# googleinterns/multimodal-long-transformer-2021

Measured on AMD Instinct MI355X. Metric: train-step samples/sec + attention TFLOPS, 4096-tok seq, higher is better.
Workload: dtype bf16; 1 GPU; BASELINE config 3: BERT-base dims, S=4096 (2+63^2 patches+125 text), radius 64 + 8 global tokens, bf16, per-GPU batch 4; step=train_step, per_gpu_batch=4, global_batch=4, seq_len=4096, parallelism=dp1, ranks_seen=1, params=111009852, optimizer=AdamW (fused flat step, bf16 shadow weights) + polynomial lr, clip 1.0, grad_allreduce=none (1 GPU), grad_reduce=mean, step_launch=HIP graph replay (recorded after 3 eager steps)

## Files before the change

include/mmt_layer.h:

```cpp
#ifndef MMT_LAYER_H_
#define MMT_LAYER_H_

#include <stddef.h>
#include <stdint.h>

#ifdef __cplusplus
extern "C" {
#endif

typedef struct mmt_rows_desc {
  int64_t rows;
  int32_t H;
  int32_t dtype;
  float eps;
  float dropout_p;
  uint64_t dropout_seed;
  int32_t accumulate;
  int32_t defer_reduce;
  const uint64_t* dropout_epoch;
} mmt_rows_desc;

size_t mmt_layer_workspace_bytes(const mmt_rows_desc* desc);

int mmt_ln_fwd(const mmt_rows_desc* desc, const void* x, const float* gamma, const float* beta,
// ... 107 lines not shown
                  void* workspace, size_t workspace_bytes, void* stream);

int mmt_embed_fwd_packed(const mmt_embed_desc* desc, const int32_t* word_ids, const int32_t* seg_ids,
                         const float* word_table, const float* seg_table, const float* pos_table ,
                         int32_t pos_rows, const float* gamma, const float* beta, const void* patch_proj ,
                         const float* patch_bias , const int32_t* example_starts,
                         const int32_t* patch_slots, int32_t n_examples, void* out, float* mean, float* rstd,
                         void* stream);
int mmt_embed_bwd_packed(const mmt_embed_desc* desc, const void* dout, const int32_t* sorted_ids,
                         const int32_t* order, const float* word_table, const float* gamma, const float* mean,
                         const float* rstd, float* dword_table, float* dgamma, float* dbeta, void* dpatch,
                         const int32_t* example_starts, const int32_t* patch_slots, int32_t n_examples,
                         void* workspace, size_t workspace_bytes, void* stream);

int mmt_xent_fwd(int64_t rows, int32_t C, int32_t dtype, const void* logits, int64_t ld,
                 const int32_t* labels, float* loss, float* lse, void* stream);
int mmt_xent_fwd_argmax(int64_t rows, int32_t C, int32_t dtype, const void* logits, int64_t ld,
                        const int32_t* labels, float* loss, float* lse, int32_t* argmax, void* stream);
int mmt_xent_bwd(int64_t rows, int32_t C, int32_t dtype, const void* logits, int64_t ld,
                 const int32_t* labels, const float* lse, const float* coef, void* dlogits, int64_t ldd,
                 void* stream);
int mmt_xent_bwd_scaled(int64_t rows, int32_t C, int32_t dtype, const void* logits, int64_t ld,
                        const int32_t* labels, const float* lse, const float* coef, const float* gscale,
                        void* dlogits, int64_t ldd, void* stream);
int mmt_weighted_loss(int64_t rows, const float* loss, const float* weight, const float* lmul, const float* mask,
                      int64_t mask_div, float* out3, float* coef, void* stream);

void mmt_ffn_set_cu_budget(int32_t cus);
int mmt_ffn_gelu_gemm(const void* x, int64_t ldx, const void* w, int64_t ldw, const float* bias, void* u,
                      int64_t ldu, void* g, int64_t ldg, int64_t M, int64_t N, int64_t K, void* stream);
int mmt_ffn_dgelu_gemm(const void* dy, int64_t lddy, const void* w, int64_t ldw, const void* u, int64_t ldu,
                       const float* bias, void* du, int64_t lddu, int64_t M, int64_t N, int64_t K, void* stream);

typedef struct mmt_image_desc {
  int32_t B;
  int32_t image_size;
  int32_t patch_size;
  int32_t out_dtype;
  int32_t channel_bits;
  float mean[3];
} mmt_image_desc;

int mmt_image_patches(const mmt_image_desc* desc, const uint8_t* pixels, int64_t pixels_bytes, const int64_t* offsets,
                      const int32_t* heights, const int32_t* widths, const uint8_t* flip, void* normalised_out,
                      float* unnormalised_out, int32_t* label_ids_out, void* stream);

#ifdef __cplusplus
}
#endif
#endif
```

multimodal-long-transformer-2021_amd/csrc/ffn_gemm.hip:

```cpp
#include "../../include/mmt_attn.h"
#include "../../include/mmt_layer.h"
#include "attn_tile.h"
#include "layer_common.h"
#include "mmt_err.h"

#include <atomic>

namespace mmt {

struct FfnGemmParams {
  const __bf16* a;
  const __bf16* b;
  const float* bias;
  const __bf16* u_in;
  __bf16* u_out;
  __bf16* d;
  long lda, ldb, ldu, ldd;
  int M, N, K, tiles_m, tiles_n, tiles_per_wg;
};

static std::atomic<int> g_ffn_cus{256};
static int cu_budget() { return g_ffn_cus.load(std::memory_order_relaxed); }

constexpr int kFfnStage = 64 * 1024;
enum { kEpiBias = 0, kEpiGelu = 1, kEpiDgelu = 2 };

__device__ __forceinline__ void ffn_wait_dma() { asm volatile("s_waitcnt vmcnt(0)" ::: "memory"); }

template <int BT, int EPI>
__global__ __launch_bounds__(512, 2) void ffn_gemm_kernel(const FfnGemmParams p) {
  extern __shared__ __attribute__((aligned(16))) unsigned char smem[];
  const int tid = threadIdx.x, lane = tid & 63;
  const int wave = __builtin_amdgcn_readfirstlane(tid >> 6);
  const int h = lane >> 5, li = lane & 15, cb = (lane >> 4) & 1, r = lane & 31;
  int t_begin, t_end;
  {
    const int nwg = gridDim.x, b = blockIdx.x, x = b & 7;
    const int base = nwg >> 3, rem = nwg & 7;
    const int L = x * base + min(x, rem) + (b >> 3);
    t_begin = L * p.tiles_per_wg;
    t_end = min(p.tiles_m * p.tiles_n, t_begin + p.tiles_per_wg);
  }
  if (t_begin >= t_end) return;
  const int n_steps = p.K >> 6;

  const bool is_a = wave < 4;
  const int drow = lane >> 3, dpos = lane & 7;
  const __bf16* gsrc[8];
#pragma unroll
  for (int j = 0; j < 8; ++j) {
    const int idx = wave * 8 + j;
    const int rg = idx & 3, row = rg * 8 + drow;
    if (idx < 32 || BT == 1) {
      const int t8 = (idx >> 2) & 7;
      const int ch = dpos ^ ((row >> 1) & 7);
      gsrc[j] = (idx < 32 ? p.a + (long)(t8 * 32 + row) * p.lda : p.b + (long)(t8 * 32 + row) * p.ldb) + ch * 8;
    } else {
      const int i2 = idx - 32, kslab = i2 >> 4, t4 = (i2 >> 2) & 3;
      const int ch = (((dpos >> 2) ^ ((row >> 1) & 1)) << 2) | (dpos & 3);
      gsrc[j] = p.b + (long)(kslab * 32 + row) * p.ldb + t4 * 64 + ch * 8;
    }
  }
  const long sstep = is_a ? 64 : (BT == 1 ? 64 : 64 * p.ldb);
  const long tstep_m = is_a ? 256 * p.lda : 0, tstep_n = is_a ? 0 : (BT == 1 ? 256 * p.ldb : 256);
  const unsigned lds0 = (unsigned)(size_t)(__attribute__((address_space(3))) unsigned char*)smem;
  auto dma = [&](unsigned stage, int tm, int tn, int step) {
    const long off = tm * tstep_m + tn * tstep_n + step * sstep;
#pragma unroll
    for (int j = 0; j < 8; ++j) glds16(gsrc[j] + off, stage + (wave * 8 + j) * 1024);
  };

  const int wm = wave & 3, wn = wave >> 2;
  const int arow = r * 128, ax = (r >> 1) & 7;
  const int frow = 8 * h + (li >> 2);
  int fo[2];
#pragma unroll
  for (int db = 0; db < 2; ++db) fo[db] = frow * 128 + ((db ^ ((frow >> 1) & 1)) << 6) + 32 * cb + 8 * (li & 3);
  const int erow = lane >> 3, ech = lane & 7;

  int tm = t_begin / p.tiles_n, tn = t_begin - tm * p.tiles_n;
  dma(lds0, tm, tn, 0);
  ffn_wait_dma();
  __syncthreads();
  int gs = 0;

  for (int t = t_begin; t < t_end; ++t) {
    int tm_next = tm, tn_next = tn + 1;
    if (tn_next == p.tiles_n) { tn_next = 0; ++tm_next; }
    f32x16 acc[2][4];
#pragma unroll
    for (int a = 0; a < 2; ++a)
#pragma unroll
      for (int b = 0; b < 4; ++b) acc[a][b] = f32x16{0};

    const int m0 = tm * 256, n0 = tn * 256;
    bf16x8 uq[3][4];
    auto load_u = [&](int blk, bf16x8 (&dst)[4]) {
      const __bf16* up = p.u_in + (long)(m0 + wm * 64 + (blk & 1) * 32 + erow) * p.ldu + n0 + wn * 128 + (blk >> 1) * 64 + ech * 8;
#pragma unroll
// ... 14 lines not shown
        for (int a = 0; a < 2; ++a)
          af[a] = *reinterpret_cast<const bf16x8*>(cur + (wm * 2 + a) * 4096 + arow + coff);
#pragma unroll
        for (int b = 0; b < 4; ++b) {
          if (BT == 1) {
            bfr[b] = *reinterpret_cast<const bf16x8*>(cur + 32768 + (wn * 4 + b) * 4096 + arow + coff);
          } else {
            const unsigned char* base = cur + 32768 + ((s >> 1) * 4 + wn * 2 + (b >> 1)) * 4096 + fo[b & 1] + (s & 1) * 2048;
            const bf16x4 lo = __builtin_bit_cast(bf16x4, __builtin_amdgcn_ds_read_tr16_b64_v4i16((__attribute__((address_space(3))) s16x4*)(base)));
            const bf16x4 hi = __builtin_bit_cast(bf16x4, __builtin_amdgcn_ds_read_tr16_b64_v4i16((__attribute__((address_space(3))) s16x4*)(base + 512)));
#pragma unroll
            for (int j = 0; j < 4; ++j) { bfr[b][j] = lo[j]; bfr[b][4 + j] = hi[j]; }
          }
        }
#pragma unroll
        for (int a = 0; a < 2; ++a)
#pragma unroll
          for (int b = 0; b < 4; ++b)
            acc[a][b] = __builtin_amdgcn_mfma_f32_32x32x16_bf16(af[a], bfr[b], acc[a][b], 0, 0, 0);
      }
      ffn_wait_dma();
      __syncthreads();
    }

    float* park = reinterpret_cast<float*>(smem + ((gs - 1) & 1) * kFfnStage + wave * 8192);
#pragma unroll
    for (int blk = 0; blk < 4; ++blk) {
      const int hb = blk >> 1, a = blk & 1;
      const int ncol = n0 + wn * 128 + hb * 64 + ech * 8;
      const int mrow0 = m0 + wm * 64 + a * 32;
      float bs[8];
#pragma unroll
      for (int j = 0; j < 8; ++j) bs[j] = 0.f;
      if (p.bias) load_param(p.bias + ncol, bs);
      if (EPI == kEpiDgelu && blk + 2 < 4) load_u(blk + 2, uq[(blk + 2) % 3]);
#pragma unroll
      for (int b2 = 0; b2 < 2; ++b2)
#pragma unroll
        for (int i = 0; i < 16; ++i) park[kap(i, h) * 64 + 32 * b2 + r] = acc[a][2 * hb + b2][i];
      __builtin_amdgcn_fence(__ATOMIC_ACQ_REL, "wavefront");
      __builtin_amdgcn_wave_barrier();
#pragma unroll
      for (int it = 0; it < 4; ++it) {
        const int row = it * 8 + erow;
        float v[8];
        Chunk<float>::load(park + row * 64 + ech * 8, v);
        const long orow = (long)(mrow0 + row);
        if (EPI == kEpiDgelu) {
          const bf16x8 uu = uq[blk % 3][it];
#pragma unroll
          for (int j = 0; j < 8; j += 2) {
            f32x2 dz;
            (void)gelu_tanh_x2(f32x2{(float)uu[j] + bs[j], (float)uu[j + 1] + bs[j + 1]}, dz);
            v[j] *= dz[0]; v[j + 1] *= dz[1];
          }
        } else {
#pragma unroll
          for (int j = 0; j < 8; ++j) v[j] += bs[j];
          if (EPI == kEpiGelu) {
            if (p.u_out) Chunk<__bf16>::store(p.u_out + orow * p.ldu + ncol, v);
#pragma unroll
            for (int j = 0; j < 8; j += 2) {
              f32x2 dz;
              const f32x2 gz = gelu_tanh_x2(f32x2{v[j], v[j + 1]}, dz);
              v[j] = gz[0]; v[j + 1] = gz[1];
            }
          }
        }
        Chunk<__bf16>::store(p.d + orow * p.ldd + ncol, v);
      }
      __builtin_amdgcn_fence(__ATOMIC_ACQ_REL, "wavefront");
      __builtin_amdgcn_wave_barrier();
    }
    if (t + 1 < t_end) __syncthreads();
    tm = tm_next; tn = tn_next;
  }
}

template <int BT, int EPI>
static hipError_t launch_ffn(const FfnGemmParams& p_in, hipStream_t st) {
  FfnGemmParams p = p_in;
  const int tiles = p.tiles_m * p.tiles_n, cus = cu_budget();
  p.tiles_per_wg = (tiles + cus - 1) / cus;
  const int grid = (tiles + p.tiles_per_wg - 1) / p.tiles_per_wg;
  const int lds = 2 * kFfnStage;
  (void)hipFuncSetAttribute(reinterpret_cast<const void*>(ffn_gemm_kernel<BT, EPI>), hipFuncAttributeMaxDynamicSharedMemorySize, lds);
  hipLaunchKernelGGL((ffn_gemm_kernel<BT, EPI>), dim3(grid), dim3(512), lds, st, p);
  return hipGetLastError();
}


static int ffn_check(const char* who, const void* a, const void* b, const void* d, int64_t M, int64_t N, int64_t K,
                     int64_t lda, int64_t ldb, int64_t ldb_min, int64_t ldd) {
  if (!a || !b || !d) return fail(MMT_E_INVALID, "%s: NULL argument", who);
  if (M <= 0 || N <= 0 || K <= 0 || (M % 256) || (N % 256) || (K % 64) || M > (1 << 30) || N > (1 << 30) || K > (1 << 30))
    return fail(MMT_E_UNSUPPORTED, "%s: needs M %% 256 == 0, N %% 256 == 0, K %% 64 == 0 (got %lld, %lld, %lld)", who,
                (long long)M, (long long)N, (long long)K);
  if ((lda % 8) || (ldb % 8) || (ldd % 8) || lda < K || ldb < ldb_min || ldd < N) return fail(MMT_E_INVALID, "%s: bad leading dimensions", who);
  if (((uintptr_t)a & 15) || ((uintptr_t)b & 15) || ((uintptr_t)d & 15)) return fail(MMT_E_INVALID, "%s: operands must be 16-byte aligned", who);
  return MMT_OK;
}

}

extern "C" void mmt_ffn_set_cu_budget(int32_t cus) {
  mmt::g_ffn_cus.store(cus < 32 ? 32 : (cus > 256 ? 256 : cus), std::memory_order_relaxed);
}

extern "C" int mmt_ffn_gelu_gemm(const void* x, int64_t ldx, const void* w, int64_t ldw, const float* bias, void* u,
                                 int64_t ldu, void* g, int64_t ldg, int64_t M, int64_t N, int64_t K, void* stream) {
  int rc = mmt::ffn_check("mmt_ffn_gelu_gemm", x, w, g, M, N, K, ldx, ldw, K, ldg);
  if (rc != MMT_OK) return rc;
  if (u && ((ldu % 8) || ldu < N || ((uintptr_t)u & 15))) return mmt::fail(MMT_E_INVALID, "mmt_ffn_gelu_gemm: bad u");
  if (bias && ((uintptr_t)bias & 15)) return mmt::fail(MMT_E_INVALID, "mmt_ffn_gelu_gemm: bias must be 16-byte aligned");
  mmt::FfnGemmParams p{};
  p.a = (const __bf16*)x; p.b = (const __bf16*)w; p.bias = bias; p.u_out = (__bf16*)u; p.d = (__bf16*)g;
  p.lda = ldx; p.ldb = ldw; p.ldu = ldu; p.ldd = ldg; p.M = (int)M; p.N = (int)N; p.K = (int)K;
  p.tiles_m = (int)(M / 256); p.tiles_n = (int)(N / 256);
  const hipError_t e = mmt::launch_ffn<1, mmt::kEpiGelu>(p, (hipStream_t)stream);
  return e == hipSuccess ? MMT_OK : mmt::fail(MMT_E_LAUNCH, "mmt_ffn_gelu_gemm: %s", hipGetErrorString(e));
}

extern "C" int mmt_ffn_dgelu_gemm(const void* dy, int64_t lddy, const void* w, int64_t ldw, const void* u, int64_t ldu,
                                  const float* bias, void* du, int64_t lddu, int64_t M, int64_t N, int64_t K, void* stream) {
  int rc = mmt::ffn_check("mmt_ffn_dgelu_gemm", dy, w, du, M, N, K, lddy, ldw, N, lddu);
  if (rc != MMT_OK) return rc;
  if (!u || (ldu % 8) || ldu < N || ((uintptr_t)u & 15)) return mmt::fail(MMT_E_INVALID, "mmt_ffn_dgelu_gemm: bad u");
  if (bias && ((uintptr_t)bias & 15)) return mmt::fail(MMT_E_INVALID, "mmt_ffn_dgelu_gemm: bias must be 16-byte aligned");
  mmt::FfnGemmParams p{};
  p.a = (const __bf16*)dy; p.b = (const __bf16*)w; p.bias = bias; p.u_in = (const __bf16*)u; p.d = (__bf16*)du;
  p.lda = lddy; p.ldb = ldw; p.ldu = ldu; p.ldd = lddu; p.M = (int)M; p.N = (int)N; p.K = (int)K;
  p.tiles_m = (int)(M / 256); p.tiles_n = (int)(N / 256);
  const hipError_t e = mmt::launch_ffn<0, mmt::kEpiDgelu>(p, (hipStream_t)stream);
  return e == hipSuccess ? MMT_OK : mmt::fail(MMT_E_LAUNCH, "mmt_ffn_dgelu_gemm: %s", hipGetErrorString(e));
}
```

multimodal-long-transformer-2021_amd/mmt_amd/_lib.py:

```python
from __future__ import annotations

import ctypes
import os
import subprocess

_HERE = os.path.dirname(os.path.abspath(__file__))
_CSRC = os.path.join(os.path.dirname(_HERE), 'csrc')
LIB_PATH = os.path.join(_HERE, 'libmmt_attn.so')

MMT_ABI_VERSION = 4
MMT_F32, MMT_BF16 = 0, 1
MMT_IDS_NONE, MMT_IDS_1D, MMT_IDS_2D = 0, 1, 2
MMT_IDS_2D_IMAGE = 3
MMT_FLAG_SCALE_BEFORE_ADD = 1
MMT_FLAG_ACCUM_REL_GRADS = 2
MMT_FLAG_EXAMPLE_IDS = 4
MMT_FLAG_EXAMPLE_STARTS = 8


def image_grid(radius: int, start: int) -> int:
  return (int(radius) & 0xFF) | ((int(start) & 0x7FFFFF) << 8)

MMT_TUNE_FWD_WALK = 0x01
MMT_TUNE_FWD_PWIN = 0x100
MMT_TUNE_FWD_ROWS_ONE_WG = 0x200
MMT_TUNE_FWD_NO_WIN = 0x02
MMT_TUNE_FWD_FORCE_WIN = 0x04
MMT_TUNE_BWD_NO_HANDOVER = 0x08
MMT_TUNE_BWD_HO_PER_WAVE = 0x10
MMT_TUNE_BWD_NO_PEEL_DQ = 0x20
MMT_TUNE_BWD_NO_PEEL_DKV = 0x40
MMT_TUNE_BWD_DQ_PLANE_MAJOR = 0x80

EXPORTS = ('mmt_abi_version', 'mmt_last_error', 'mmt_write_step_scalars', 'mmt_workspace_bytes', 'mmt_attn_fwd',
           'mmt_attn_bwd', 'mmt_side_inputs',
           'mmt_layer_workspace_bytes', 'mmt_ln_fwd', 'mmt_ln_bwd', 'mmt_residual_block_fwd',
           'mmt_residual_block_bwd', 'mmt_bias_gelu_fwd', 'mmt_bias_gelu_bwd', 'mmt_colsum_reduce', 'mmt_colsum_reduce_batch', 'mmt_accumulate_grad', 'mmt_grad_clip_scale', 'mmt_adamw_step', 'mmt_wgrad_accumulate',
           'mmt_wgrad_bias_accumulate', 'mmt_wgrad_grouped', 'mmt_wgrad_group_workspace_bytes', 'mmt_wgrad_workspace_bytes', 'mmt_wgrad_set_cu_budget', 'mmt_embed_fwd', 'mmt_embed_bwd', 'mmt_embed_fwd_packed', 'mmt_embed_bwd_packed',
           'mmt_embed_workspace_bytes', 'mmt_xent_fwd', 'mmt_xent_fwd_argmax', 'mmt_xent_bwd', 'mmt_xent_bwd_scaled', 'mmt_weighted_loss', 'mmt_colsum', 'mmt_colsum_workspace_bytes', 'mmt_ln_bwd_add', 'mmt_ffn_gelu_gemm', 'mmt_ffn_dgelu_gemm', 'mmt_ffn_set_cu_budget',
           'mmt_image_patches')


class EmbedDesc(ctypes.Structure):
  _fields_ = [('rows', ctypes.c_int64), ('S', ctypes.c_int32), ('H', ctypes.c_int32), ('dtype', ctypes.c_int32),
              ('vocab', ctypes.c_int32), ('seg_vocab', ctypes.c_int32), ('patch_start', ctypes.c_int32),
              ('n_patch', ctypes.c_int32), ('eps', ctypes.c_float), ('dropout_p', ctypes.c_float),
              ('accumulate', ctypes.c_int32), ('dropout_seed', ctypes.c_uint64), ('dropout_epoch', ctypes.c_void_p)]


class RowsDesc(ctypes.Structure):
  _fields_ = [('rows', ctypes.c_int64), ('H', ctypes.c_int32), ('dtype', ctypes.c_int32),
              ('eps', ctypes.c_float), ('dropout_p', ctypes.c_float),
              ('dropout_seed', ctypes.c_uint64), ('accumulate', ctypes.c_int32),
              ('defer_reduce', ctypes.c_int32), ('dropout_epoch', ctypes.c_void_p)]


class MaskDesc(ctypes.Structure):
  _fields_ = [('valid_len', ctypes.c_void_p), ('local_radius', ctypes.c_int32),
              ('global_start', ctypes.c_int32), ('n_global', ctypes.c_int32),
              ('id_mode', ctypes.c_int32), ('max_dist', ctypes.c_int32),
              ('patches_per_row', ctypes.c_int32), ('core_layers', ctypes.c_int32),
              ('image_grid', ctypes.c_int32), ('global_index', ctypes.c_void_p)]


class AttnDesc(ctypes.Structure):
  _fields_ = [('B', ctypes.c_int32), ('S', ctypes.c_int32), ('N', ctypes.c_int32),
              ('D', ctypes.c_int32), ('R', ctypes.c_int32), ('dtype', ctypes.c_int32),
              ('q_stride', ctypes.c_int64 * 3), ('k_stride', ctypes.c_int64 * 3),
              ('v_stride', ctypes.c_int64 * 3), ('o_stride', ctypes.c_int64 * 3),
              ('scale', ctypes.c_float), ('mask_value', ctypes.c_float),
              ('flags', ctypes.c_uint32), ('dropout_p', ctypes.c_float),
              ('dropout_seed', ctypes.c_uint64), ('mask', MaskDesc),
# ... 102 lines not shown
  ed = ctypes.POINTER(EmbedDesc)
  L.mmt_embed_fwd.restype = ctypes.c_int
  L.mmt_embed_fwd.argtypes = [ed] + [vp] * 13
  L.mmt_embed_bwd.restype = ctypes.c_int
  L.mmt_embed_bwd.argtypes = [ed] + [vp] * 12 + [ctypes.c_size_t, vp]
  L.mmt_embed_fwd_packed.restype = ctypes.c_int
  L.mmt_embed_fwd_packed.argtypes = [ed] + [vp] * 5 + [ctypes.c_int32] + [vp] * 6 + [ctypes.c_int32] + [vp] * 4
  L.mmt_embed_bwd_packed.restype = ctypes.c_int
  L.mmt_embed_bwd_packed.argtypes = [ed] + [vp] * 13 + [ctypes.c_int32, vp, ctypes.c_size_t, vp]
  L.mmt_embed_workspace_bytes.restype = ctypes.c_size_t
  L.mmt_embed_workspace_bytes.argtypes = [ed]
  L.mmt_xent_fwd_argmax.restype = ctypes.c_int
  L.mmt_xent_fwd_argmax.argtypes = [ctypes.c_int64, ctypes.c_int32, ctypes.c_int32, vp, ctypes.c_int64, vp, vp, vp, vp, vp]
  L.mmt_xent_fwd.restype = ctypes.c_int
  L.mmt_xent_fwd.argtypes = [ctypes.c_int64, ctypes.c_int32, ctypes.c_int32, vp, ctypes.c_int64, vp, vp, vp, vp]
  L.mmt_colsum_workspace_bytes.restype = ctypes.c_size_t
  L.mmt_colsum_workspace_bytes.argtypes = [ctypes.c_int64, ctypes.c_int32]
  L.mmt_colsum.restype = ctypes.c_int
  L.mmt_colsum.argtypes = [ctypes.c_int64, ctypes.c_int32, ctypes.c_int32, vp, ctypes.c_int64, vp, ctypes.c_int32, vp,
                           ctypes.c_size_t, vp]
  L.mmt_xent_bwd_scaled.restype = ctypes.c_int
  L.mmt_xent_bwd_scaled.argtypes = [ctypes.c_int64, ctypes.c_int32, ctypes.c_int32, vp, ctypes.c_int64, vp, vp, vp, vp,
                                    vp, ctypes.c_int64, vp]
  L.mmt_weighted_loss.restype = ctypes.c_int
  L.mmt_weighted_loss.argtypes = [ctypes.c_int64, vp, vp, vp, vp, ctypes.c_int64, vp, vp, vp]
  L.mmt_xent_bwd.restype = ctypes.c_int
  L.mmt_xent_bwd.argtypes = [ctypes.c_int64, ctypes.c_int32, ctypes.c_int32, vp, ctypes.c_int64, vp, vp, vp, vp,
                             ctypes.c_int64, vp]
  i64 = ctypes.c_int64
  L.mmt_ffn_gelu_gemm.restype = ctypes.c_int
  L.mmt_ffn_gelu_gemm.argtypes = [vp, i64, vp, i64, vp, vp, i64, vp, i64, i64, i64, i64, vp]
  L.mmt_ffn_dgelu_gemm.restype = ctypes.c_int
  L.mmt_ffn_dgelu_gemm.argtypes = [vp, i64, vp, i64, vp, i64, vp, vp, i64, i64, i64, i64, vp]
  L.mmt_ffn_set_cu_budget.restype = None
  L.mmt_ffn_set_cu_budget.argtypes = [ctypes.c_int32]
  L.mmt_wgrad_set_cu_budget.restype = None
  L.mmt_wgrad_set_cu_budget.argtypes = [ctypes.c_int32]
  L.mmt_wgrad_workspace_bytes.restype = ctypes.c_size_t
  L.mmt_wgrad_workspace_bytes.argtypes = [ctypes.c_int32, ctypes.c_int32, ctypes.c_int64]
  L.mmt_adamw_step.restype = ctypes.c_int
  L.mmt_adamw_step.argtypes = [ctypes.POINTER(AdamwDesc)] + [vp] * 8
  L.mmt_grad_clip_scale.restype = ctypes.c_int
  L.mmt_grad_clip_scale.argtypes = [ctypes.c_int32, ctypes.POINTER(ctypes.c_void_p), ctypes.POINTER(ctypes.c_int64), ctypes.c_float,
                                    ctypes.c_float, vp, vp, vp, ctypes.c_size_t, vp]
  L.mmt_accumulate_grad.restype = ctypes.c_int
  L.mmt_accumulate_grad.argtypes = [vp, vp, ctypes.c_int32, ctypes.c_int64, vp]
  L.mmt_image_patches.restype = ctypes.c_int
  L.mmt_image_patches.argtypes = [ctypes.POINTER(ImageDesc), vp, i64, vp, vp, vp, vp, vp, vp, vp, vp]
  L.mmt_write_step_scalars.restype = ctypes.c_int
  L.mmt_write_step_scalars.argtypes = [vp, vp, ctypes.c_uint64, ctypes.c_float, ctypes.c_float, ctypes.c_float, vp]
  if L.mmt_abi_version() != MMT_ABI_VERSION:
    raise ImportError('libmmt_attn ABI version mismatch')
  _lib = L
  return L


def check(rc: int) -> None:
  if rc != 0:
    raise MmtError(rc, lib().mmt_last_error().decode())
```

multimodal-long-transformer-2021_amd/mmt_amd/fused.py:

```python
from __future__ import annotations


from typing import Optional

import torch

from . import _lib, step_scalars

_seed_state = {'base': 0, 'n': 0}


def set_seed_stream(step: int, micro_step: int = 0, rank: int = 0) -> None:
  _seed_state['base'] = ((int(micro_step) * 0xC2B2AE3D27D4EB4F) ^ ((int(rank) + 1) * 0x165667B19E3779F9)) & ((1 << 63) - 1)
  _seed_state['n'] = 0
  step_scalars.set_step(step)


def next_seed(base: int = 0) -> int:
  _seed_state['n'] += 1
  return (_seed_state['base'] + int(base) * 0x9E3779B97F4A7C15
          + _seed_state['n'] * 0xD1B54A32D192ED03) & ((1 << 63) - 1)


def _desc(x2d: torch.Tensor, eps=1e-12, p=0.0, seed=0) -> _lib.RowsDesc:
# ... 300 lines not shown

def _ffn_gemm_ok(a: torch.Tensor, w: torch.Tensor, M: int, N: int, K: int) -> bool:
  return (a.is_cuda and a.dtype == torch.bfloat16 and w.dtype == torch.bfloat16 and M % 256 == 0 and N % 256 == 0
          and K % 64 == 0 and a.stride(1) == 1 and w.stride(1) == 1 and a.stride(0) % 8 == 0 and w.stride(0) % 8 == 0
          and a.data_ptr() % 16 == 0 and w.data_ptr() % 16 == 0)


def ffn_gelu_gemm(x: torch.Tensor, w: torch.Tensor, bias: Optional[torch.Tensor]):
  M, K = x.shape
  N = w.shape[0]
  if not (w.shape[1] == K and _ffn_gemm_ok(x, w, M, N, K)
          and (bias is None or (bias.dtype == torch.float32 and bias.is_contiguous() and bias.numel() == N))):
    return None
  u = torch.empty(M, N, device=x.device, dtype=torch.bfloat16)
  g = torch.empty_like(u)
  with torch.cuda.device(x.device):
    _lib.check(_lib.lib().mmt_ffn_gelu_gemm(_p(x), x.stride(0), _p(w), w.stride(0), _p(bias) if bias is not None else None,
                                            _p(u), N, _p(g), N, M, N, K, _stream(x)))
  return u, g


def ffn_dgelu_gemm(dy: torch.Tensor, w: torch.Tensor, u: torch.Tensor, bias: Optional[torch.Tensor] = None):
  M, K = dy.shape
  N = w.shape[1]
  if not (w.shape[0] == K and u.shape == (M, N) and u.dtype == torch.bfloat16 and u.stride(1) == 1
          and u.stride(0) % 8 == 0 and u.data_ptr() % 16 == 0 and _ffn_gemm_ok(dy, w, M, N, K)
          and (bias is None or (bias.dtype == torch.float32 and bias.is_contiguous() and bias.numel() == N))):
    return None
  du = torch.empty(M, N, device=dy.device, dtype=torch.bfloat16)
  with torch.cuda.device(dy.device):
    _lib.check(_lib.lib().mmt_ffn_dgelu_gemm(_p(dy), dy.stride(0), _p(w), w.stride(0), _p(u), u.stride(0),
                                             _p(bias) if bias is not None else None, _p(du), N, M, N, K, _stream(dy)))
  return du

def colsum(x2: torch.Tensor, out: Optional[torch.Tensor] = None) -> torch.Tensor:
  if not (x2.is_cuda and x2.dim() == 2 and x2.stride(1) == 1 and x2.dtype in (torch.float32, torch.bfloat16)
          and x2.shape[0] > 0 and x2.shape[1] > 0):
    s = x2.sum(0, dtype=torch.float32)
    return s if out is None else out.add_(s)
  rows, C = x2.shape
  L = _lib.lib()
  ws = torch.empty(max(L.mmt_colsum_workspace_bytes(rows, C), 16), dtype=torch.uint8, device=x2.device)
  acc = out is not None
  if acc and (out.dtype != torch.float32 or not out.is_contiguous() or out.numel() != C):
    raise ValueError('colsum: out must be a contiguous fp32 [C] tensor')
  res = out if acc else torch.empty(C, dtype=torch.float32, device=x2.device)
  with torch.cuda.device(x2.device):
    _lib.check(L.mmt_colsum(rows, C, _dtype_code(x2.dtype), _p(x2), x2.stride(0), _p(res), int(acc), _p(ws), ws.numel(),
                            _stream(x2)))
  return res


def accumulate_grad_(acc: torch.Tensor, g: torch.Tensor) -> torch.Tensor:
  if (not acc.is_cuda or acc.dtype != torch.float32 or not acc.is_contiguous() or not g.is_contiguous()
      or g.dtype not in (torch.float32, torch.bfloat16) or acc.numel() != g.numel()
      or acc.data_ptr() % 16 or g.data_ptr() % 16):
    return acc.add_(g)
  code = _lib.MMT_F32 if g.dtype == torch.float32 else _lib.MMT_BF16
  with torch.cuda.device(acc.device):
    _lib.check(_lib.lib().mmt_accumulate_grad(acc.data_ptr(), g.data_ptr(), code, acc.numel(), _stream(acc)))
  return acc


def wgrad_accumulate_(dw: torch.Tensor, dy: torch.Tensor, x: torch.Tensor, dbias: Optional[torch.Tensor] = None) -> bool:
  K, M = dy.shape
  N = x.shape[1]
# ... 260 lines not shown
        local = (_arange_i32(S, dout.device).long().repeat(B) - st).clamp_(0, S - 1).clamp_(max=pos_table.shape[0] - 1)
        dpos.index_add_(0, local, dout2.float())
      dpos = dpos.to(pos_table.dtype)
    return (None, None, dword_ret, dseg, dpos, _finish(gamma, dg, direct), _finish(beta, db, direct), dpatch, None)


def embed_assemble(word_ids, seg_ids, word_table, seg_table, gamma, beta, pos_table=None, patch_proj=None,
                   eps=1e-12, p=0.0, seed=0, patch_start=2, out_dtype=torch.bfloat16, example_starts=None,
                   patch_slots=None):
  return _EmbedAssembleFn.apply(word_ids, seg_ids, word_table, seg_table, pos_table, gamma, beta, patch_proj,
                                (eps, p, seed, patch_start, out_dtype, example_starts, patch_slots))


class _SoftmaxXentFn(torch.autograd.Function):

  @staticmethod
  def forward(ctx, logits, labels):
    _check(logits, labels)
    rows, C = logits.shape
    lab = labels.reshape(-1).to(torch.int32).contiguous()
    loss = torch.empty(rows, dtype=torch.float32, device=logits.device)
    lse = torch.empty_like(loss)
    with torch.cuda.device(logits.device):
      _lib.check(_lib.lib().mmt_xent_fwd(rows, C, _dtype_code(logits.dtype), _p(logits), logits.stride(0), _p(lab),
                                         _p(loss), _p(lse), _stream(logits)))
    ctx.save_for_backward(logits, lab, lse)
    return loss

  @staticmethod
  def backward(ctx, dloss):
    logits, lab, lse = ctx.saved_tensors
    rows, C = logits.shape
    coef = dloss.to(torch.float32).contiguous()
    dlogits = torch.empty_like(logits)
    with torch.cuda.device(logits.device):
      _lib.check(_lib.lib().mmt_xent_bwd(rows, C, _dtype_code(logits.dtype), _p(logits), logits.stride(0), _p(lab),
                                         _p(lse), _p(coef), _p(dlogits), dlogits.stride(0), _stream(logits)))
    return dlogits, None


class _WeightedXentFn(torch.autograd.Function):

  @staticmethod
  def forward(ctx, logits, labels, weight, lmul, mask, mask_div, want_argmax=False):
    rows, C = logits.shape
    dev = logits.device
    lab = labels.reshape(-1).to(torch.int32).contiguous()
    w = weight.reshape(-1).to(torch.float32).contiguous()
    lm = None if lmul is None else lmul.reshape(-1).to(torch.float32).contiguous()
    mk = None if mask is None else mask.reshape(-1).to(torch.float32).contiguous()
    buf = torch.empty(3 * rows + 3, dtype=torch.float32, device=dev)
    loss, lse, coef, out3 = buf[:rows], buf[rows:2 * rows], buf[2 * rows:3 * rows], buf[3 * rows:]
    amax = torch.empty(rows, dtype=torch.int32, device=dev) if want_argmax else None
    with torch.cuda.device(dev):
      _lib.check(_lib.lib().mmt_xent_fwd_argmax(rows, C, _dtype_code(logits.dtype), _p(logits), logits.stride(0), _p(lab),
                                                _p(loss), _p(lse), _p(amax) if want_argmax else None, _stream(logits)))
      _lib.check(_lib.lib().mmt_weighted_loss(rows, _p(loss), _p(w), _p(lm) if lm is not None else None,
                                              _p(mk) if mk is not None else None, int(mask_div), _p(out3), _p(coef),
                                              _stream(logits)))
    ctx.save_for_backward(logits, lab, buf)
    if want_argmax:
      ctx.mark_non_differentiable(amax)
      return out3[0], amax
    return out3[0]

  @staticmethod
  def backward(ctx, dloss, *_unused):
    logits, lab, buf = ctx.saved_tensors
    rows, C = logits.shape
    lse, coef = buf[rows:2 * rows], buf[2 * rows:3 * rows]
    g = dloss.reshape(1).to(torch.float32)
    dlogits = torch.empty_like(logits)
    with torch.cuda.device(logits.device):
      _lib.check(_lib.lib().mmt_xent_bwd_scaled(rows, C, _dtype_code(logits.dtype), _p(logits), logits.stride(0), _p(lab),
                                                _p(lse), _p(coef), _p(g), _p(dlogits), dlogits.stride(0), _stream(logits)))
    return dlogits, None, None, None, None, None, None


def weighted_softmax_cross_entropy(logits, labels, weight, lmul=None, mask=None, mask_div=1, return_argmax=False):
  if logits.dim() != 2 or logits.stride(1) != 1 or not 0 < logits.shape[0] <= 65535:
    raise ValueError('weighted_softmax_cross_entropy expects [0 < rows <= 65535, C] logits with unit column stride')
  _check(logits, labels)
  return _WeightedXentFn.apply(logits, labels, weight, lmul, mask, mask_div, bool(return_argmax))


def softmax_cross_entropy(logits: torch.Tensor, labels: torch.Tensor) -> torch.Tensor:
  if logits.dim() != 2 or logits.stride(1) != 1 or logits.shape[0] > 65535:
    raise ValueError('softmax_cross_entropy expects [rows <= 65535, C] logits with unit column stride')
  return _SoftmaxXentFn.apply(logits, labels)
```

multimodal-long-transformer-2021_amd/mmt_amd/layers.py:

```python
from __future__ import annotations

import math
from typing import Callable, Optional

import torch
import torch.nn as nn
import torch.nn.functional as F

from . import fused, ops


def truncated_normal_(t: torch.Tensor, stddev: float) -> torch.Tensor:
  return nn.init.trunc_normal_(t, mean=0.0, std=stddev, a=-2 * stddev, b=2 * stddev)


def _GELU_TANH(x):
  return F.gelu(x, approximate='tanh')


def get_activation(name_or_fn) -> Optional[Callable]:
  if name_or_fn is None or callable(name_or_fn):
    return name_or_fn
  table = {'gelu': _GELU_TANH, 'relu': F.relu, 'tanh': torch.tanh,
           'linear': None, 'identity': None}
# ... 135 lines not shown
  def backward(ctx, df):
    x2, u, g, w1s, w2s = ctx.saved_tensors
    w1, b1, w2 = ctx.params
    df2 = df.reshape(-1, df.shape[-1])
    if not df2.is_contiguous():
      df2 = df2.contiguous()
    _accumulate_dense_grads(w2, None, df2, g)
    du = fused.ffn_dgelu_gemm(df2, w2s, u, b1.detach())
    if du is None:
      raise RuntimeError('mmt_ffn_dgelu_gemm refused a shape _ffn_ok admitted')
    _accumulate_dense_grads(w1, b1, du, x2)
    dx = torch.mm(du, w1s).view(ctx.shape) if ctx.needs_input_grad[0] else None
    return dx, None, None, None


def _ffn_ok(x, w1, b1, w2) -> bool:
  return (x.is_cuda and x.dtype == torch.bfloat16 and torch.is_grad_enabled()
          and all(isinstance(t, nn.Parameter) and t.dtype == torch.float32 for t in (w1, b1, w2))
          and x.numel() // x.shape[-1] % 256 == 0 and w1.shape[0] % 256 == 0 and x.shape[-1] % 64 == 0)


def _linear(x: torch.Tensor, weight: torch.Tensor, bias: Optional[torch.Tensor]) -> torch.Tensor:
  if (x.is_cuda and x.dtype == torch.bfloat16 and torch.is_grad_enabled() and isinstance(weight, nn.Parameter)
      and weight.dtype == torch.float32 and (bias is None or isinstance(bias, nn.Parameter))):
    return _LinearFn.apply(x, weight, bias)
  return F.linear(x, cast_param(weight, x.dtype), None if bias is None else cast_param(bias, x.dtype))




class _TiedLogitsFn(torch.autograd.Function):

  @staticmethod
  def forward(ctx, x, table, bias):
    w = _param_weight(table, x.dtype)
    b = None if bias is None else _param_weight(bias, x.dtype)
    ctx.save_for_backward(x, w)
    ctx.params = (table, bias)
    return F.linear(x, w, b)

  @staticmethod
  def backward(ctx, dy):
    x, w = ctx.saved_tensors
    table, bias = ctx.params
    dx = None
    if ctx.needs_input_grad[0]:
      M, V = dy.shape
      if (dy.is_cuda and dy.dtype == torch.bfloat16 and dy.is_contiguous() and w.is_contiguous()
          and V % 3 == 0 and V >= 8192 and M * w.shape[1] <= (1 << 21)):
        k = V // 3
        dx = torch.bmm(dy.as_strided((3, M, k), (k, V, 1)), w.view(3, k, w.shape[1])).sum(0, dtype=torch.float32).to(dy.dtype)
      else:
        dx = torch.mm(dy, w)
    if table.requires_grad:
      if table.grad is None:
        table.grad = torch.zeros_like(table, dtype=torch.float32)
      fused.accumulate_grad_(table.grad, torch.mm(dy.t(), x))
    db = None
    if bias is not None and bias.requires_grad:
      db = (fused.colsum(dy) if dy.is_cuda else dy.sum(0, dtype=torch.float32)).to(bias.dtype)
    return dx, None, db


class EmbeddingLookup(nn.Module):

  def __init__(self, vocab_size: int, embedding_size: int, projection_size: Optional[int] = None,
               initializer_range: float = 0.02, use_one_hot_lookup: bool = False, name: str = ''):
    super().__init__()
    self.vocab_size, self.embedding_size = vocab_size, embedding_size
    self.projection_size = projection_size
    self.initializer_range = initializer_range
    self.use_one_hot_lookup = use_one_hot_lookup
    self.name = name
    self.embedding_table = nn.Parameter(torch.empty(vocab_size, embedding_size))
    truncated_normal_(self.embedding_table, initializer_range)
    if projection_size is not None and projection_size != embedding_size:
      self.embedding_projection = nn.Parameter(torch.empty(projection_size, embedding_size))
      truncated_normal_(self.embedding_projection, initializer_range)
    else:
      self.embedding_projection = None

  def forward(self, ids: torch.Tensor) -> torch.Tensor:
    out = F.embedding(ids.long(), self.embedding_table)
    if self.embedding_projection is not None:
# ... 345 lines not shown
```

Measured before the change: 269.6 samples/s.

## Add custom padded-vocab logits GEMM and split-K dgrad kernel for tied MLM head

Routes the tied vocabulary logits projection through the custom FFN GEMM kernel, with a VOC mode that clamps rows past the vocabulary and writes logits into a buffer whose leading dimension is rounded up to 256. The backward dgrad (dlogits × table) becomes a split-K pass over the padded vocab that writes fp32 slabs, followed by a separate reduce kernel. The cross-entropy backward now allocates a padded dlogits buffer so the fast path can take it. The goal is to replace the rocBLAS/bmm path on the odd-sized vocab GEMMs with better-tiled kernels that fill the CUs. In exchange it adds an fp32 workspace, an extra reduce launch and padding traffic.

```diff
diff --git a/include/mmt_layer.h b/include/mmt_layer.h
--- a/include/mmt_layer.h
+++ b/include/mmt_layer.h
@@ -163,6 +163,12 @@
 int mmt_ffn_dgelu_gemm(const void* dy, int64_t lddy, const void* w, int64_t ldw, const void* u, int64_t ldu,
                        const float* bias, void* du, int64_t lddu, int64_t M, int64_t N, int64_t K, void* stream);
 
+int mmt_vocab_logits(const void* x, int64_t ldx, const void* table, int64_t ldt, const float* bias, void* logits,
+                     int64_t ldv, int64_t M, int64_t V, int64_t H, void* stream);
+size_t mmt_vocab_dgrad_workspace_bytes(int64_t M, int64_t V, int64_t H);
+int mmt_vocab_dgrad(const void* dlogits, int64_t ldv, const void* table, int64_t ldt, void* dx, int64_t M, int64_t V,
+                    int64_t H, void* workspace, size_t workspace_bytes, void* stream);
+
 typedef struct mmt_image_desc {
   int32_t B;
   int32_t image_size;
diff --git a/multimodal-long-transformer-2021_amd/csrc/ffn_gemm.hip b/multimodal-long-transformer-2021_amd/csrc/ffn_gemm.hip
--- a/multimodal-long-transformer-2021_amd/csrc/ffn_gemm.hip
+++ b/multimodal-long-transformer-2021_amd/csrc/ffn_gemm.hip
@@ -17,17 +17,19 @@
   __bf16* d;
   long lda, ldb, ldu, ldd;
   int M, N, K, tiles_m, tiles_n, tiles_per_wg;
+  int b_rows, n_valid, split, steps_per_slice;
+  float* slabs;
 };
 
 static std::atomic<int> g_ffn_cus{256};
 static int cu_budget() { return g_ffn_cus.load(std::memory_order_relaxed); }
 
 constexpr int kFfnStage = 64 * 1024;
-enum { kEpiBias = 0, kEpiGelu = 1, kEpiDgelu = 2 };
+enum { kEpiBias = 0, kEpiGelu = 1, kEpiDgelu = 2, kEpiSlab = 3 };
 
 __device__ __forceinline__ void ffn_wait_dma() { asm volatile("s_waitcnt vmcnt(0)" ::: "memory"); }
 
-template <int BT, int EPI>
+template <int BT, int EPI, int VOC = 0>
 __global__ __launch_bounds__(512, 2) void ffn_gemm_kernel(const FfnGemmParams p) {
   extern __shared__ __attribute__((aligned(16))) unsigned char smem[];
   const int tid = threadIdx.x, lane = tid & 63;
@@ -39,10 +41,17 @@
     const int base = nwg >> 3, rem = nwg & 7;
     const int L = x * base + min(x, rem) + (b >> 3);
     t_begin = L * p.tiles_per_wg;
-    t_end = min(p.tiles_m * p.tiles_n, t_begin + p.tiles_per_wg);
+    t_end = min(p.tiles_m * p.tiles_n * (VOC ? p.split : 1), t_begin + p.tiles_per_wg);
   }
   if (t_begin >= t_end) return;
-  const int n_steps = p.K >> 6;
+  int n_steps = p.K >> 6, ks = 0, step0 = 0;
+  if (VOC) {
+    const int tiles = p.tiles_m * p.tiles_n;
+    ks = t_begin / tiles;
+    t_begin -= ks * tiles; t_end -= ks * tiles;
+    step0 = ks * p.steps_per_slice;
+    n_steps = min(p.steps_per_slice, n_steps - step0);
+  }
 
   const bool is_a = wave < 4;
   const int drow = lane >> 3, dpos = lane & 7;
@@ -65,6 +74,27 @@
   const long tstep_m = is_a ? 256 * p.lda : 0, tstep_n = is_a ? 0 : (BT == 1 ? 256 * p.ldb : 256);
   const unsigned lds0 = (unsigned)(size_t)(__attribute__((address_space(3))) unsigned char*)smem;
   auto dma = [&](unsigned stage, int tm, int tn, int step) {
+    step += step0;
+    if (VOC) {
+      const __bf16* base = is_a ? p.a : p.b;
+      const long ld = is_a ? p.lda : p.ldb;
+      const int row_max = is_a ? p.M - 1 : p.b_rows - 1;
+#pragma unroll
+      for (int j = 0; j < 8; ++j) {
+        const int idx = wave * 8 + j, row = (idx & 3) * 8 + drow;
+        int grow; long gcol;
+        if (BT == 1 || is_a) {
+          grow = (is_a ? tm : tn) * 256 + ((idx >> 2) & 7) * 32 + row;
+          gcol = step * 64 + (dpos ^ ((row >> 1) & 7)) * 8;
+        } else {
+          const int i2 = idx - 32;
+          grow = step * 64 + (i2 >> 4) * 32 + row;
+          gcol = tn * 256 + ((i2 >> 2) & 3) * 64 + ((((dpos >> 2) ^ ((row >> 1) & 1)) << 2) | (dpos & 3)) * 8;
+        }
+        glds16(base + (long)min(grow, row_max) * ld + gcol, __builtin_amdgcn_readfirstlane(stage + (wave * 8 + j) * 1024));
+      }
+      return;
+    }
     const long off = tm * tstep_m + tn * tstep_n + step * sstep;
 #pragma unroll
     for (int j = 0; j < 8; ++j) glds16(gsrc[j] + off, stage + (wave * 8 + j) * 1024);
@@ -145,7 +175,14 @@
       float bs[8];
 #pragma unroll
       for (int j = 0; j < 8; ++j) bs[j] = 0.f;
-      if (p.bias) load_param(p.bias + ncol, bs);
+      if (VOC) {
+        if (EPI == kEpiBias && p.bias) {
+          if (ncol + 8 <= p.n_valid) load_param(p.bias + ncol, bs);
+          else
+#pragma unroll
+            for (int j = 0; j < 8; ++j) if (ncol + j < p.n_valid) bs[j] = p.bias[ncol + j];
+        }
+      } else if (p.bias) load_param(p.bias + ncol, bs);
       if (EPI == kEpiDgelu && blk + 2 < 4) load_u(blk + 2, uq[(blk + 2) % 3]);
 #pragma unroll
       for (int b2 = 0; b2 < 2; ++b2)
@@ -159,6 +196,10 @@
         float v[8];
         Chunk<float>::load(park + row * 64 + ech * 8, v);
         const long orow = (long)(mrow0 + row);
+        if (EPI == kEpiSlab) {
+          Chunk<float>::store(p.slabs + ((long)ks * p.M + orow) * p.N + ncol, v);
+          continue;
+        }
         if (EPI == kEpiDgelu) {
           const bf16x8 uu = uq[blk % 3][it];
 #pragma unroll
@@ -180,6 +221,9 @@
             }
           }
         }
+        if (VOC && ncol + 8 > p.n_valid)
+#pragma unroll
+          for (int j = 0; j < 8; ++j) if (ncol + j >= p.n_valid) v[j] = 0.f;
         Chunk<__bf16>::store(p.d + orow * p.ldd + ncol, v);
       }
       __builtin_amdgcn_fence(__ATOMIC_ACQ_REL, "wavefront");
@@ -190,16 +234,38 @@
   }
 }
 
-template <int BT, int EPI>
+template <int BT, int EPI, int VOC = 0>
 static hipError_t launch_ffn(const FfnGemmParams& p_in, hipStream_t st) {
   FfnGemmParams p = p_in;
-  const int tiles = p.tiles_m * p.tiles_n, cus = cu_budget();
-  p.tiles_per_wg = (tiles + cus - 1) / cus;
+  const int tiles = p.tiles_m * p.tiles_n * (VOC ? p.split : 1), cus = cu_budget();
+  p.tiles_per_wg = (VOC && p.split > 1) ? 1 : (tiles + cus - 1) / cus;
   const int grid = (tiles + p.tiles_per_wg - 1) / p.tiles_per_wg;
   const int lds = 2 * kFfnStage;
-  (void)hipFuncSetAttribute(reinterpret_cast<const void*>(ffn_gemm_kernel<BT, EPI>), hipFuncAttributeMaxDynamicSharedMemorySize, lds);
-  hipLaunchKernelGGL((ffn_gemm_kernel<BT, EPI>), dim3(grid), dim3(512), lds, st, p);
+  (void)hipFuncSetAttribute(reinterpret_cast<const void*>(ffn_gemm_kernel<BT, EPI, VOC>), hipFuncAttributeMaxDynamicSharedMemorySize, lds);
+  hipLaunchKernelGGL((ffn_gemm_kernel<BT, EPI, VOC>), dim3(grid), dim3(512), lds, st, p);
   return hipGetLastError();
+}
+
+__global__ __launch_bounds__(256) void vocab_reduce_kernel(const float* slabs, int split, long n, __bf16* out) {
+  const long e = ((long)blockIdx.x * 256 + threadIdx.x) * 8;
+  if (e >= n) return;
+  float a[8];
+  Chunk<float>::load(slabs + e, a);
+  for (int s2 = 1; s2 < split; ++s2) {
+    float b[8];
+    Chunk<float>::load(slabs + (long)s2 * n + e, b);
+#pragma unroll
+    for (int j = 0; j < 8; ++j) a[j] += b[j];
+  }
+  Chunk<__bf16>::store(out + e, a);
+}
+
+static int vocab_dgrad_split(int tiles, int steps, int& steps_per_slice) {
+  int split = cu_budget() / tiles;
+  if (split > steps / 4) split = steps / 4;
+  if (split < 1) split = 1;
+  steps_per_slice = (steps + split - 1) / split;
+  return (steps + steps_per_slice - 1) / steps_per_slice;
 }
 
 
@@ -247,3 +313,59 @@
   const hipError_t e = mmt::launch_ffn<0, mmt::kEpiDgelu>(p, (hipStream_t)stream);
   return e == hipSuccess ? MMT_OK : mmt::fail(MMT_E_LAUNCH, "mmt_ffn_dgelu_gemm: %s", hipGetErrorString(e));
 }
+
+static int vocab_check(const char* who, const void* a, const void* tab, const void* d, int64_t M, int64_t V, int64_t H,
+                       int64_t ldv, int64_t ldt, int64_t ldx) {
+  if (!a || !tab || !d) return mmt::fail(MMT_E_INVALID, "%s: NULL argument", who);
+  if (M <= 0 || V <= 0 || H <= 0 || (M % 256) || (H % 256) || M > (1 << 30) || V > (1 << 30) - 256 || H > (1 << 30))
+    return mmt::fail(MMT_E_UNSUPPORTED, "%s: needs M %% 256 == 0, H %% 256 == 0 (got M = %lld, V = %lld, H = %lld)", who,
+                     (long long)M, (long long)V, (long long)H);
+  if (ldv != (V + 255) / 256 * 256 || (ldt % 8) || ldt < H || (ldx % 8) || ldx < H)
+    return mmt::fail(MMT_E_INVALID, "%s: ldv must be V rounded up to 256, table and x strides multiples of 8 and >= H", who);
+  if (((uintptr_t)a & 15) || ((uintptr_t)tab & 15) || ((uintptr_t)d & 15)) return mmt::fail(MMT_E_INVALID, "%s: operands must be 16-byte aligned", who);
+  return MMT_OK;
+}
+
+extern "C" int mmt_vocab_logits(const void* x, int64_t ldx, const void* table, int64_t ldt, const float* bias, void* logits,
+                                int64_t ldv, int64_t M, int64_t V, int64_t H, void* stream) {
+  int rc = vocab_check("mmt_vocab_logits", x, table, logits, M, V, H, ldv, ldt, ldx);
+  if (rc != MMT_OK) return rc;
+  if (bias && ((uintptr_t)bias & 15)) return mmt::fail(MMT_E_INVALID, "mmt_vocab_logits: bias must be 16-byte aligned");
+  mmt::FfnGemmParams p{};
+  p.a = (const __bf16*)x; p.b = (const __bf16*)table; p.bias = bias; p.d = (__bf16*)logits;
+  p.lda = ldx; p.ldb = ldt; p.ldd = ldv; p.M = (int)M; p.N = (int)ldv; p.K = (int)H;
+  p.tiles_m = (int)(M / 256); p.tiles_n = (int)(ldv / 256);
+  p.b_rows = (int)V; p.n_valid = (int)V; p.split = 1; p.steps_per_slice = (int)(H / 64);
+  const hipError_t e = mmt::launch_ffn<1, mmt::kEpiBias, 1>(p, (hipStream_t)stream);
+  return e == hipSuccess ? MMT_OK : mmt::fail(MMT_E_LAUNCH, "mmt_vocab_logits: %s", hipGetErrorString(e));
+}
+
+extern "C" size_t mmt_vocab_dgrad_workspace_bytes(int64_t M, int64_t V, int64_t H) {
+  if (M <= 0 || V <= 0 || H <= 0 || (M % 256) || (H % 256) || M > (1 << 30) || V > (1 << 30) - 256 || H > (1 << 30)) return 0;
+  int sps;
+  const int split = mmt::vocab_dgrad_split((int)(M / 256 * (H / 256)), (int)((V + 255) / 256 * 4), sps);
+  return (size_t)split * M * H * sizeof(float);
+}
+
+extern "C" int mmt_vocab_dgrad(const void* dlogits, int64_t ldv, const void* table, int64_t ldt, void* dx, int64_t M,
+                               int64_t V, int64_t H, void* workspace, size_t workspace_bytes, void* stream) {
+  int rc = vocab_check("mmt_vocab_dgrad", dlogits, table, dx, M, V, H, ldv, ldt, H);
+  if (rc != MMT_OK) return rc;
+  const size_t need = mmt_vocab_dgrad_workspace_bytes(M, V, H);
+  if (!workspace || workspace_bytes < need || ((uintptr_t)workspace & 15))
+    return mmt::fail(MMT_E_WORKSPACE, "mmt_vocab_dgrad: workspace too small: need %zu bytes, got %zu", need, workspace_bytes);
+  mmt::FfnGemmParams p{};
+  p.a = (const __bf16*)dlogits; p.b = (const __bf16*)table; p.slabs = (float*)workspace;
+  p.lda = ldv; p.ldb = ldt; p.M = (int)M; p.N = (int)H; p.K = (int)ldv;
+  p.tiles_m = (int)(M / 256); p.tiles_n = (int)(H / 256);
+  p.b_rows = (int)V; p.n_valid = (int)H;
+  p.split = mmt::vocab_dgrad_split(p.tiles_m * p.tiles_n, (int)(ldv / 64), p.steps_per_slice);
+  hipStream_t st = (hipStream_t)stream;
+  hipError_t e = mmt::launch_ffn<0, mmt::kEpiSlab, 1>(p, st);
+  if (e == hipSuccess) {
+    const long n = (long)M * H;
+    hipLaunchKernelGGL(mmt::vocab_reduce_kernel, dim3((unsigned)((n / 8 + 255) / 256)), dim3(256), 0, st, p.slabs, p.split, n, (__bf16*)dx);
+    e = hipGetLastError();
+  }
+  return e == hipSuccess ? MMT_OK : mmt::fail(MMT_E_LAUNCH, "mmt_vocab_dgrad: %s", hipGetErrorString(e));
+}
diff --git a/multimodal-long-transformer-2021_amd/mmt_amd/_lib.py b/multimodal-long-transformer-2021_amd/mmt_amd/_lib.py
--- a/multimodal-long-transformer-2021_amd/mmt_amd/_lib.py
+++ b/multimodal-long-transformer-2021_amd/mmt_amd/_lib.py
@@ -38,6 +38,7 @@
            'mmt_residual_block_bwd', 'mmt_bias_gelu_fwd', 'mmt_bias_gelu_bwd', 'mmt_colsum_reduce', 'mmt_colsum_reduce_batch', 'mmt_accumulate_grad', 'mmt_grad_clip_scale', 'mmt_adamw_step', 'mmt_wgrad_accumulate',
            'mmt_wgrad_bias_accumulate', 'mmt_wgrad_grouped', 'mmt_wgrad_group_workspace_bytes', 'mmt_wgrad_workspace_bytes', 'mmt_wgrad_set_cu_budget', 'mmt_embed_fwd', 'mmt_embed_bwd', 'mmt_embed_fwd_packed', 'mmt_embed_bwd_packed',
            'mmt_embed_workspace_bytes', 'mmt_xent_fwd', 'mmt_xent_fwd_argmax', 'mmt_xent_bwd', 'mmt_xent_bwd_scaled', 'mmt_weighted_loss', 'mmt_colsum', 'mmt_colsum_workspace_bytes', 'mmt_ln_bwd_add', 'mmt_ffn_gelu_gemm', 'mmt_ffn_dgelu_gemm', 'mmt_ffn_set_cu_budget',
+           'mmt_vocab_logits', 'mmt_vocab_dgrad', 'mmt_vocab_dgrad_workspace_bytes',
            'mmt_image_patches')
 
 
@@ -206,6 +207,12 @@
   L.mmt_ffn_gelu_gemm.argtypes = [vp, i64, vp, i64, vp, vp, i64, vp, i64, i64, i64, i64, vp]
   L.mmt_ffn_dgelu_gemm.restype = ctypes.c_int
   L.mmt_ffn_dgelu_gemm.argtypes = [vp, i64, vp, i64, vp, i64, vp, vp, i64, i64, i64, i64, vp]
+  L.mmt_vocab_logits.restype = ctypes.c_int
+  L.mmt_vocab_logits.argtypes = [vp, i64, vp, i64, vp, vp, i64, i64, i64, i64, vp]
+  L.mmt_vocab_dgrad_workspace_bytes.restype = ctypes.c_size_t
+  L.mmt_vocab_dgrad_workspace_bytes.argtypes = [i64, i64, i64]
+  L.mmt_vocab_dgrad.restype = ctypes.c_int
+  L.mmt_vocab_dgrad.argtypes = [vp, i64, vp, i64, vp, i64, i64, i64, vp, ctypes.c_size_t, vp]
   L.mmt_ffn_set_cu_budget.restype = None
   L.mmt_ffn_set_cu_budget.argtypes = [ctypes.c_int32]
   L.mmt_wgrad_set_cu_budget.restype = None
diff --git a/multimodal-long-transformer-2021_amd/mmt_amd/fused.py b/multimodal-long-transformer-2021_amd/mmt_amd/fused.py
--- a/multimodal-long-transformer-2021_amd/mmt_amd/fused.py
+++ b/multimodal-long-transformer-2021_amd/mmt_amd/fused.py
@@ -356,6 +356,62 @@
     _lib.check(_lib.lib().mmt_ffn_dgelu_gemm(_p(dy), dy.stride(0), _p(w), w.stride(0), _p(u), u.stride(0),
                                              _p(bias) if bias is not None else None, _p(du), N, M, N, K, _stream(dy)))
   return du
+
+def vocab_ld(V: int) -> int:
+  return (V + 255) // 256 * 256
+
+
+def is_vocab_padded(t: torch.Tensor) -> bool:
+  if not (t.is_cuda and t.dim() == 2 and t.dtype == torch.bfloat16 and t.shape[0] > 0 and t.shape[1] > 0):
+    return False
+  M, V = t.shape
+  ldv = vocab_ld(V)
+  return (t.stride(1) == 1 and t.stride(0) == ldv and t.data_ptr() % 16 == 0
+          and (t.storage_offset() + M * ldv) * t.element_size() <= t.untyped_storage().nbytes())
+
+
+def vocab_padded_like(t: torch.Tensor) -> torch.Tensor:
+  if not is_vocab_padded(t) or t.stride(0) == t.shape[1]:
+    return torch.empty_like(t)
+  M, V = t.shape
+  buf = torch.empty(M, t.stride(0), dtype=t.dtype, device=t.device)
+  buf[:, V:].zero_()
+  return buf[:, :V]
+
+
+def _vocab_ok(x, table, M, V, H) -> bool:
+  return (x.is_cuda and x.dtype == torch.bfloat16 and table.dtype == torch.bfloat16 and table.device == x.device
+          and x.dim() == 2 and table.shape == (V, H) and x.shape == (M, H) and M % 256 == 0 and H % 256 == 0
+          and x.is_contiguous() and table.is_contiguous() and x.data_ptr() % 16 == 0 and table.data_ptr() % 16 == 0)
+
+
+def vocab_logits(x: torch.Tensor, table: torch.Tensor, bias: Optional[torch.Tensor]):
+  M, H = x.shape
+  V = table.shape[0]
+  if not (_vocab_ok(x, table, M, V, H)
+          and (bias is None or (bias.dtype == torch.float32 and bias.is_contiguous() and bias.numel() == V
+                                and bias.data_ptr() % 16 == 0))):
+    return None
+  ldv = vocab_ld(V)
+  buf = torch.empty(M, ldv, dtype=torch.bfloat16, device=x.device)
+  with torch.cuda.device(x.device):
+    _lib.check(_lib.lib().mmt_vocab_logits(_p(x), H, _p(table), H, _p(bias), _p(buf), ldv, M, V, H, _stream(x)))
+  return buf[:, :V]
+
+
+def vocab_dgrad(dy: torch.Tensor, table: torch.Tensor):
+  M, V = dy.shape
+  H = table.shape[1]
+  if not (is_vocab_padded(dy) and table.dtype == torch.bfloat16 and table.shape[0] == V and table.is_contiguous()
+          and table.data_ptr() % 16 == 0 and table.device == dy.device and M % 256 == 0 and H % 256 == 0):
+    return None
+  L = _lib.lib()
+  ws = torch.empty(max(L.mmt_vocab_dgrad_workspace_bytes(M, V, H), 16), dtype=torch.uint8, device=dy.device)
+  dx = torch.empty(M, H, dtype=torch.bfloat16, device=dy.device)
+  with torch.cuda.device(dy.device):
+    _lib.check(L.mmt_vocab_dgrad(_p(dy), dy.stride(0), _p(table), H, _p(dx), M, V, H, _p(ws), ws.numel(), _stream(dy)))
+  return dx
+
 
 def colsum(x2: torch.Tensor, out: Optional[torch.Tensor] = None) -> torch.Tensor:
   if not (x2.is_cuda and x2.dim() == 2 and x2.stride(1) == 1 and x2.dtype in (torch.float32, torch.bfloat16)
@@ -682,7 +738,7 @@
     logits, lab, lse = ctx.saved_tensors
     rows, C = logits.shape
     coef = dloss.to(torch.float32).contiguous()
-    dlogits = torch.empty_like(logits)
+    dlogits = vocab_padded_like(logits)
     with torch.cuda.device(logits.device):
       _lib.check(_lib.lib().mmt_xent_bwd(rows, C, _dtype_code(logits.dtype), _p(logits), logits.stride(0), _p(lab),
                                          _p(lse), _p(coef), _p(dlogits), dlogits.stride(0), _stream(logits)))
@@ -720,7 +776,7 @@
     rows, C = logits.shape
     lse, coef = buf[rows:2 * rows], buf[2 * rows:3 * rows]
     g = dloss.reshape(1).to(torch.float32)
-    dlogits = torch.empty_like(logits)
+    dlogits = vocab_padded_like(logits)
     with torch.cuda.device(logits.device):
       _lib.check(_lib.lib().mmt_xent_bwd_scaled(rows, C, _dtype_code(logits.dtype), _p(logits), logits.stride(0), _p(lab),
                                                 _p(lse), _p(coef), _p(g), _p(dlogits), dlogits.stride(0), _stream(logits)))
diff --git a/multimodal-long-transformer-2021_amd/mmt_amd/layers.py b/multimodal-long-transformer-2021_amd/mmt_amd/layers.py
--- a/multimodal-long-transformer-2021_amd/mmt_amd/layers.py
+++ b/multimodal-long-transformer-2021_amd/mmt_amd/layers.py
@@ -191,11 +191,22 @@
 class _TiedLogitsFn(torch.autograd.Function):
 
   @staticmethod
+  def _vocab_path(x, table, w, bias) -> bool:
+    return (x.is_cuda and x.dtype == torch.bfloat16 and x.dim() == 2 and x.shape[0] % 256 == 0 and x.shape[1] % 256 == 0
+            and table.dtype == torch.float32 and w.dtype == torch.bfloat16 and w.is_contiguous() and x.is_contiguous()
+            and (bias is None or (bias.dtype == torch.float32 and bias.is_contiguous())))
+
+  @staticmethod
   def forward(ctx, x, table, bias):
     w = _param_weight(table, x.dtype)
+    ctx.params = (table, bias)
+    if _TiedLogitsFn._vocab_path(x, table, w, bias):
+      logits = fused.vocab_logits(x, w, None if bias is None else bias.detach())
+      if logits is not None:
+        ctx.save_for_backward(x, w)
+        return logits
     b = None if bias is None else _param_weight(bias, x.dtype)
     ctx.save_for_backward(x, w)
-    ctx.params = (table, bias)
     return F.linear(x, w, b)
 
   @staticmethod
@@ -203,12 +214,17 @@
     x, w = ctx.saved_tensors
     table, bias = ctx.params
     dx = None
+    vocab = fused.is_vocab_padded(dy) and _TiedLogitsFn._vocab_path(x, table, w, None)
     if ctx.needs_input_grad[0]:
       M, V = dy.shape
-      if (dy.is_cuda and dy.dtype == torch.bfloat16 and dy.is_contiguous() and w.is_contiguous()
+      if vocab:
+        dx = fused.vocab_dgrad(dy, w)
+      if dx is not None:
+        pass
+      elif (dy.is_cuda and dy.dtype == torch.bfloat16 and dy.stride(1) == 1 and w.is_contiguous()
           and V % 3 == 0 and V >= 8192 and M * w.shape[1] <= (1 << 21)):
         k = V // 3
-        dx = torch.bmm(dy.as_strided((3, M, k), (k, V, 1)), w.view(3, k, w.shape[1])).sum(0, dtype=torch.float32).to(dy.dtype)
+        dx = torch.bmm(dy.as_strided((3, M, k), (k, dy.stride(0), 1)), w.view(3, k, w.shape[1])).sum(0, dtype=torch.float32).to(dy.dtype)
       else:
         dx = torch.mm(dy, w)
     if table.requires_grad:
```

New measurement: 270.8 samples/s, median of 6. About the same (+0.4%).
